# deep-privacy/SA-toolkit

Measured on AMD Instinct MI355X. Metric: anonymized audio seconds per wall-clock second (real-time factor), 5 s @ 16 kHz utterances, higher is better.
Workload: dtype f32 (matrix products as split-f16: hi*hi on the f16 MFMA; cross terms on the block-scaled 8-bit MFMA (weights e4m3, activations e5m2) in the ResBlock convs of stages [1, 2] = 51 % of the generator's FLOP, as two more f16 products elsewhere; f32 accumulate)

## Files before the change

sa-toolkit_amd/csrc/conv1d_mfma.hip:

```cpp
#include "common.h"
#include "conv_common.h"
#include <cstring>

namespace sat {

static int g_k1_gemm = 3;
static int g_lean3 = 1, g_lean7 = 1, g_lean11 = 1;
static int g_trim_halo = 1;
static int g_half_tile7 = 1;
static int g_pair32s = 1;

template <int MT, int NT, int WM, int WN, int KS, bool STRIDE1, int XWI>
__global__ void __launch_bounds__(256, 2) conv1d_mfma_kernel(const ConvArgs p) {
  extern __shared__ __attribute__((aligned(16))) float lds[];
  constexpr int CO_B = 32 * MT * WM;
  constexpr int T_B = 32 * NT * WN;
  static_assert(WM * WN == 4, "4 waves per block");

  const int tid = threadIdx.x;
  const int lane = tid & 63;
  const int wave = tid >> 6;
  const int wm = wave % WM;
  const int wn = wave / WM;
  const int l31 = lane & 31;
// ... 1799 lines not shown
extern "C" int sat_resblock_pair_scaled_f16x3(const sat_conv1d_desc* d, const float* x, const void* w1_packed,
                                              const float* bias1, float w1_descale, const void* w2_packed, float* y, void* stream) {
  SAT_REQUIRE(d && w1_packed && w2_packed && bias1 && d->bias && (x || d->x_split) && (y || (d->no_y && d->y_split)),
              "resblock_pair: null pointer");
  SAT_REQUIRE(d->C_in == d->C_out && d->C_in % 16 == 0 &&
                  (d->C_in <= 32 || (d->C_in == 64 && d->x_split && d->res_split)),
              "resblock_pair: C must be 16 or 32 (64 with 3 taps and split planes end to end)");
  SAT_REQUIRE(d->groups == 1 && d->up == 1 && d->stride == 1 && d->T_q == d->T_in, "resblock_pair: same-length conv pair only");
  SAT_REQUIRE(d->ksize == 3 || d->ksize == 7 || d->ksize == 11, "resblock_pair: kernel size %d not instantiated", d->ksize);
  SAT_REQUIRE(d->in_lrelu, "resblock_pair: both convs take a leaky-relu input");
  SAT_REQUIRE((d->res && d->res == x && !d->res_split) || (!d->res && d->res_split && d->res_split == d->x_split),
              "resblock_pair: the residual is the block input (res == x, or res_split == x_split)");
  ConvArgs a{};
  a.x = x;
  a.w = (const float*)w1_packed;
  a.w2 = w2_packed;
  a.bias1 = bias1;
  a.y = y;
  a.bias = d->bias;
  a.res = d->res;
  a.x_bs = d->x_bstride; a.x_cs = d->x_cstride;
  a.y_bs = d->y_bstride; a.y_cs = d->y_cstride;
  a.r_bs = d->res_bstride; a.r_cs = d->res_cstride;
  a.cin_g = d->C_in; a.cout_g = d->C_out; a.rows_g = d->C_out;
  a.T_in = d->T_in; a.T_q = d->T_q;
  a.ksize = d->ksize; a.dil = d->dilation; a.stride = 1; a.up = 1;
  a.pad_left = (d->ksize * d->dilation - d->dilation) / 2;
  a.cin_pad = round_up(a.cin_g, CI_CHUNK);
  a.co_pad = 64;
  a.w_gs = (long long)(a.cin_pad / CI_CHUNK) * a.ksize * a.co_pad * 64;
  a.in_lrelu = 1; a.in_slope = d->in_slope;
  SAT_REQUIRE(d->in_slope >= 0.f && d->in_slope <= 1.f && (!d->y_split || (d->y_split_slope >= 0.f && d->y_split_slope <= 1.f)) &&
                  (!d->res_split || d->res_split_slope <= 1.f),
              "resblock_pair: leaky-relu slopes must lie in [0, 1] (common.h lrelu_max)");
  a.accum = d->accum; a.accum_div = d->accum_div;
  a.no_store = d->accum_no_store;
  SAT_REQUIRE(!d->accum_no_store || (d->accum && y && d->y_split && !d->no_y), "resblock_pair: accum_no_store goes with accum and y_split");
  a.res_scale = 1.f; a.res_toff = 0; a.res_tstride = 1;
  a.w_descale = d->w_descale != 0.f ? d->w_descale : 1.f;
  a.w_descale1 = w1_descale != 0.f ? w1_descale : 1.f;
  SAT_REQUIRE((long long)a.cin_g * a.x_cs * 4 < (1LL << 31) && (long long)a.rows_g * a.y_cs * 4 < (1LL << 31),
              "resblock_pair: slab too large for 31-bit offsets");
  a.fast_epi = 1;
  a.x16 = d->x_split;
  a.y16 = d->y_split;
  a.y16_slope = d->y_split_slope;
  a.no_y = d->no_y;
  SAT_REQUIRE(!(d->no_y && d->accum), "resblock_pair: no_y with accum");
  if (a.no_y) a.y = (float*)a.y16;
  if (d->res_split) {
    SAT_REQUIRE(d->res_split_slope > 0.f, "resblock_pair: res_split_slope");
    a.res16 = d->res_split;
    a.res16_inv = 1.0f / d->res_split_slope;
  }
  SAT_REQUIRE((long long)a.rows_g * a.T_q * 4 < (1LL << 31), "resblock_pair: slab too large");
  hipStream_t s = (hipStream_t)stream;
  if (a.cin_g == 16 && a.x16 && a.res16) {
    switch (a.ksize) {
      case 3: return launch_pair16<3>(a, d->B, s);
      case 7: return launch_pair16<7>(a, d->B, s);
      default: return launch_pair16<11>(a, d->B, s);
    }
  }
  if (a.cin_g == 64 && g_pair32s && pair32s_supports(a)) return launch_pair32s(a, d->B, s);
  if (a.cin_g == 64) {
    SAT_REQUIRE(pair64_supports(a), "resblock_pair(C = 64): split planes in, residual from planes, (ksize - 1) * dilation <= 64");
    a.xw = g_trim_halo ? 128 + (a.ksize - 1) * a.dil : 192;
    return launch_pair64(a, d->B, s);
  }
  if (a.cin_g == 32 && a.x16 && a.res16) {
    if (g_pair32s && pair32s_supports(a)) return launch_pair32s(a, d->B, s);
    switch (a.ksize) {
      case 3: return launch_pair32<3>(a, d->B, s);
      case 7: return launch_pair32<7>(a, d->B, s);
      default: return launch_pair32<11>(a, d->B, s);
    }
  }
  switch (a.ksize) {
    case 3: return launch_pair<3>(a, d->B, s);
    case 7: return launch_pair<7>(a, d->B, s);
    default: return launch_pair<11>(a, d->B, s);
  }
}

extern "C" int sat_conv1d_f8r_supported(const sat_conv1d_desc* d) {
  if (!d || d->mode != SAT_CONV_F16F8R || !d->x_split || !d->x_split8 || d->groups != 1) return 0;
  ConvArgs a;
  float dummy;
  if (conv1d_prepare(d, nullptr, &dummy, d->no_y ? nullptr : &dummy, a) != SAT_OK) return 0;
  return convring_supports(a, d->B) ? 1 : 0;
}

__global__ void __launch_bounds__(256) planes_f8_sidecar_kernel(const uint4* __restrict__ x, uint4* __restrict__ y, int C, int T) {
  const int t = blockIdx.x * 256 + threadIdx.x;
  const int chunk = blockIdx.y, b = blockIdx.z;
  if (t >= T) return;
  const uint4* xb = x + ((long long)b * (C / 16) + chunk) * 4 * T + t;
  typedef _Float16 h8v __attribute__((ext_vector_type(8)));
  const h8v h0 = __builtin_bit_cast(h8v, xb[0]), h1 = __builtin_bit_cast(h8v, xb[T]);
  const h8v l0 = __builtin_bit_cast(h8v, xb[2LL * T]), l1 = __builtin_bit_cast(h8v, xb[3LL * T]);
  uint4 oh, ol;
  oh.x = pack_e5m2x4((float)h0[0], (float)h0[1], (float)h0[2], (float)h0[3]);
  oh.y = pack_e5m2x4((float)h0[4], (float)h0[5], (float)h0[6], (float)h0[7]);
  oh.z = pack_e5m2x4((float)h1[0], (float)h1[1], (float)h1[2], (float)h1[3]);
  oh.w = pack_e5m2x4((float)h1[4], (float)h1[5], (float)h1[6], (float)h1[7]);
  const float k = F8_XLO_SCALE;
  ol.x = pack_e5m2x4((float)l0[0] * k, (float)l0[1] * k, (float)l0[2] * k, (float)l0[3] * k);
  ol.y = pack_e5m2x4((float)l0[4] * k, (float)l0[5] * k, (float)l0[6] * k, (float)l0[7] * k);
  ol.z = pack_e5m2x4((float)l1[0] * k, (float)l1[1] * k, (float)l1[2] * k, (float)l1[3] * k);
  ol.w = pack_e5m2x4((float)l1[4] * k, (float)l1[5] * k, (float)l1[6] * k, (float)l1[7] * k);
  uint4* yb = y + ((long long)b * (C / 16) + chunk) * 2 * T + t;
  yb[0] = oh;
  yb[T] = ol;
}

extern "C" int sat_planes_f8_sidecar(const void* x_split, void* x_split8, int B, int C, int T, void* stream) {
  SAT_REQUIRE(x_split && x_split8, "planes_f8_sidecar: null pointer");
  SAT_REQUIRE(B > 0 && C > 0 && T > 0 && C % 16 == 0 && B < 65536 && C / 16 < 65536, "planes_f8_sidecar: unsupported shape B=%d C=%d T=%d", B, C, T);
  dim3 grid(ceil_div(T, 256), C / 16, B);
  hipLaunchKernelGGL(planes_f8_sidecar_kernel, grid, dim3(256), 0, (hipStream_t)stream, (const uint4*)x_split, (uint4*)x_split8, C, T);
  SAT_LAUNCH_CHECK("planes_f8_sidecar_kernel");
  return SAT_OK;
}

extern "C" int sat_act_split_f32(const float* x, void* x_split, int B, int C, int T, float slope, int format, void* stream) {
  SAT_REQUIRE(x && x_split, "act_split: null pointer");
  SAT_REQUIRE(format == SAT_SPLIT_F16 || format == SAT_SPLIT_F8, "act_split: unknown format");
  SAT_REQUIRE(B > 0 && C > 0 && T > 0 && C % 16 == 0 && B < 65536, "act_split: unsupported shape B=%d C=%d T=%d", B, C, T);
  SAT_REQUIRE(slope >= 0.f && slope <= 1.f, "act_split: slope must lie in [0, 1]");
  dim3 grid(ceil_div(T, 256), C / 8, B);
  hipLaunchKernelGGL(act_split_kernel, grid, dim3(256), 0, (hipStream_t)stream, x, (uint4*)x_split, C, T, slope, format == SAT_SPLIT_F8);
  SAT_LAUNCH_CHECK("act_split_kernel");
  return SAT_OK;
}

extern "C" int sat_pair32_debug_stamps(int64_t* buf) { return pair32_debug_stamps((long long*)buf); }
extern "C" int sat_convring_debug_stamps(int64_t* buf) { return convring_debug_stamps((long long*)buf); }

extern "C" int sat_conv_set_option(const char* name, int value) {
  SAT_REQUIRE(name, "conv_set_option: null name");
  if (!strcmp(name, "lean3")) { g_lean3 = value != 0; return SAT_OK; }
  if (!strcmp(name, "lean7")) { g_lean7 = value != 0; return SAT_OK; }
  if (!strcmp(name, "lean11")) { g_lean11 = value != 0; return SAT_OK; }
  if (!strcmp(name, "half_tile7")) { g_half_tile7 = value != 0; return SAT_OK; }
  if (!strcmp(name, "pair32s")) { g_pair32s = value != 0; return SAT_OK; }
  if (!strcmp(name, "trim_halo")) { g_trim_halo = value != 0; return SAT_OK; }
  if (!strcmp(name, "pair32w")) { pair32w_set(value); return SAT_OK; }
  if (!strcmp(name, "pair64w")) { pair64w_set(value); return SAT_OK; }
  if (!strcmp(name, "pair64_rpre")) { pair64_rpre_set(value); return SAT_OK; }
  if (!strcmp(name, "convpost_quad")) { convpost_set_quad(value); return SAT_OK; }
  if (!strcmp(name, "convring")) { convring_set(value); return SAT_OK; }
  if (!strcmp(name, "convring_blocks")) { convring_set_blocks(value); return SAT_OK; }
  if (!strcmp(name, "convring_wr")) { convring_set_wr(value); return SAT_OK; }
  if (!strcmp(name, "gemm_walk")) { gemm_walk_set(value); return SAT_OK; }
  if (!strcmp(name, "lean_balance")) { lean_set_balance(value); return SAT_OK; }
  if (!strcmp(name, "pair32s_waves")) { pair32s_set_waves(value); return SAT_OK; }
  if (!strcmp(name, "k1_gemm")) { g_k1_gemm = value < 0 ? 0 : value > 3 ? 3 : value; return SAT_OK; }
  set_error("conv_set_option: unknown option '%s'", name);
  return SAT_ERR_INVALID;
}
```

sa-toolkit_amd/csrc/conv_common.h:

```cpp
#pragma once
#include "common.h"

namespace sat {


typedef float f32x16 __attribute__((ext_vector_type(16)));

typedef int i32x8 __attribute__((ext_vector_type(8)));
typedef _Float16 h8 __attribute__((ext_vector_type(8)));

constexpr float F8_XLO_SCALE = 1024.f;
constexpr int F8_E_XHI = 127, F8_E_XLO = 127 - 10, F8_E_WHI = 127 - 6, F8_E_WLO = 127 - 16;
constexpr int F8R_E_WHI = 127 + 2, F8R_E_WLO = 127 - 9;

__device__ __forceinline__ unsigned pack_e4m3x4(float a, float b, float c, float d) {
  a = __builtin_amdgcn_fmed3f(a, -448.f, 448.f);
  b = __builtin_amdgcn_fmed3f(b, -448.f, 448.f);
  c = __builtin_amdgcn_fmed3f(c, -448.f, 448.f);
  d = __builtin_amdgcn_fmed3f(d, -448.f, 448.f);
  int w = __builtin_amdgcn_cvt_pk_fp8_f32(a, b, 0, false);
  w = __builtin_amdgcn_cvt_pk_fp8_f32(c, d, w, true);
  return (unsigned)w;
}

// ... 441 lines not shown
  const __amdgpu_buffer_rsrc_t scs = __builtin_amdgcn_make_buffer_rsrc((void*)(p.ch_scale ? p.ch_scale : p.y), 0, p.ch_scale ? chn : 0u, 0x00020000);
  const __amdgpu_buffer_rsrc_t shs = __builtin_amdgcn_make_buffer_rsrc((void*)(p.ch_shift ? p.ch_shift : p.y), 0, p.ch_shift ? chn : 0u, 0x00020000);
  const __amdgpu_buffer_rsrc_t y16rs = __builtin_amdgcn_make_buffer_rsrc(
      (void*)(p.y16 ? (char*)p.y16 + (long long)b * p.rows_g * p.T_q * 4 : (char*)p.y), 0,
      p.y16 ? (unsigned)(p.rows_g * p.T_q * 4) : 0u, 0x00020000);
  const int y_rb = (int)p.y_cs * 4;
  const bool has_res = p.res != nullptr || p.res16 != nullptr;
  float bi[MT][4], sc[MT][4], sh[MT][4];
#pragma unroll
  for (int m = 0; m < MT; ++m) {
    const int row0 = co_w + m * 16 + 4 * lg;
#pragma unroll
    for (int r = 0; r < 4; ++r) bi[m][r] = __builtin_bit_cast(float, __builtin_amdgcn_raw_buffer_load_b32(brs, (row0 + r) * 4, 0, 0));
  }
  if (HAS_BN && p.ch_scale) {
#pragma unroll
    for (int m = 0; m < MT; ++m) {
      const int row0 = co_w + m * 16 + 4 * lg;
#pragma unroll
      for (int r = 0; r < 4; ++r) {
        sc[m][r] = __builtin_bit_cast(float, __builtin_amdgcn_raw_buffer_load_b32(scs, (row0 + r) * 4, 0, 0));
        sh[m][r] = __builtin_bit_cast(float, __builtin_amdgcn_raw_buffer_load_b32(shs, (row0 + r) * 4, 0, 0));
      }
    }
  }
  f32x4 yn[NT];
  auto load_accum = [&](int m) __attribute__((always_inline)) {
    const int row0 = co_w + m * 16 + 4 * lg;
#pragma unroll
    for (int n = 0; n < NT; ++n) {
      const int q = q_w + n * 16 + li;
      const unsigned yoff = q < p.T_q ? (unsigned)(row0 * y_rb + q * 4) : OOB;
#pragma unroll
      for (int r = 0; r < 4; ++r) yn[n][r] = __builtin_bit_cast(float, __builtin_amdgcn_raw_buffer_load_b32(yrs, yoff + r * y_rb, 0, 0));
    }
  };
  f32x4 rn[NT];
  if (ROWRES && has_res) epilogue16_load_res_row<NT>(p, rn, b, co_w, q_w, li, lg);
  if (p.accum) load_accum(0);
#pragma unroll
  for (int m = 0; m < MT; ++m) {
    const int row0 = co_w + m * 16 + 4 * lg;
    const bool rows_ok = co_w + m * 16 < p.rows_g;
    f32x4 yv[NT], rr[NT];
    if (ROWRES && has_res) {
#pragma unroll
      for (int n = 0; n < NT; ++n) rr[n] = rn[n];
      if (m + 1 < MT) epilogue16_load_res_row<NT>(p, rn, b, co_w + 16 * (m + 1), q_w, li, lg);
    }
    if (p.accum) {
#pragma unroll
      for (int n = 0; n < NT; ++n) yv[n] = yn[n];
      if (m + 1 < MT) load_accum(m + 1);
    }
#pragma unroll
    for (int n = 0; n < NT; ++n) {
      const int q = q_w + n * 16 + li;
      const bool qok = q < p.T_q;
      const unsigned yoff = qok ? (unsigned)(row0 * y_rb + q * 4) : OOB;
      float rv[4], v[4];
      const f32x4 rw = ROWRES ? rr[n] : rpre[m][n];
      if (p.res16) {
        decode_res16(rw[0], rw[1], rw[2], rw[3], p.res16_inv, rv);
      } else if (p.res) {
#pragma unroll
        for (int r = 0; r < 4; ++r) rv[r] = rw[r];
      }
#pragma unroll
      for (int r = 0; r < 4; ++r) v[r] = __builtin_fmaf(acc[m][n][r], p.w_descale, bi[m][r]);
      if (has_res && !p.res_after) {
#pragma unroll
        for (int r = 0; r < 4; ++r) v[r] += p.res_scale * rv[r];
      }
      if (p.relu && p.relu_first) {
#pragma unroll
        for (int r = 0; r < 4; ++r) v[r] = v[r] > 0.f ? v[r] : 0.f;
      }
      if (HAS_BN && p.ch_scale) {
#pragma unroll
        for (int r = 0; r < 4; ++r) v[r] = v[r] * sc[m][r] + sh[m][r];
      }
      if (p.relu && !p.relu_first) {
#pragma unroll
        for (int r = 0; r < 4; ++r) v[r] = v[r] > 0.f ? v[r] : 0.f;
      }
      if (p.gelu) gelu_fast4(v);
      if (has_res && p.res_after) {
#pragma unroll
        for (int r = 0; r < 4; ++r) v[r] += p.res_scale * rv[r];
      }
      if (p.accum) {
#pragma unroll
        for (int r = 0; r < 4; ++r) v[r] = yv[n][r] + v[r];
      }
      if (p.accum_div != 0.f) {
#pragma unroll
        for (int r = 0; r < 4; ++r) v[r] = v[r] / p.accum_div;
      }
      if (!p.no_y && !p.no_store) {
#pragma unroll
        for (int r = 0; r < 4; ++r)
          __builtin_amdgcn_raw_buffer_store_b32(__builtin_bit_cast(unsigned, v[r]), yrs, yoff + r * y_rb, 0, 0);
      }
      if (p.y16 && rows_ok) {
        const int chunk = (co_w >> 4) + m;
        float u[4];
#pragma unroll
        for (int r = 0; r < 4; ++r) u[r] = lrelu_max(v[r], p.y16_slope);
        const auto h01 = __builtin_amdgcn_cvt_pkrtz(u[0], u[1]);
        const auto h23 = __builtin_amdgcn_cvt_pkrtz(u[2], u[3]);
        const auto l01 = split_lo2(h01, u[0], u[1]);
        const auto l23 = split_lo2(h23, u[2], u[3]);
        const unsigned off = qok ? (unsigned)(((chunk * 4 + (lg >> 1)) * p.T_q + q) * 16 + 8 * (lg & 1)) : OOB;
        typedef unsigned u32x2 __attribute__((ext_vector_type(2)));
        u32x2 hv, lv;
        hv[0] = __builtin_bit_cast(unsigned, h01); hv[1] = __builtin_bit_cast(unsigned, h23);
        lv[0] = __builtin_bit_cast(unsigned, l01); lv[1] = __builtin_bit_cast(unsigned, l23);
        __builtin_amdgcn_raw_buffer_store_b64(hv, y16rs, off, 0, 0);
        __builtin_amdgcn_raw_buffer_store_b64(lv, y16rs, off, 2 * p.T_q * 16, 0);
      }
    }
  }
}

inline bool epilogue16_supports(const ConvArgs& a) {
  return a.fast_epi && !a.y16_f8 && a.up == 1 && !a.poly_planes && a.rows_g % 4 == 0;
}

int launch_f16x3_ring(const ConvArgs& a, int B, hipStream_t s);
int launch_pair64(const ConvArgs& a, int B, hipStream_t s);
bool pair64_supports(const ConvArgs& a);
int launch_pair32s(const ConvArgs& a, int B, hipStream_t s);
bool pair32s_supports(const ConvArgs& a);
void lean_set_balance(int v);
void pair32s_set_waves(int n);
void pair32w_set(int v);
void pair64w_set(int v);
void pair64_rpre_set(int v);
int pair32_debug_stamps(long long* buf);
int launch_f16x3_lean(const ConvArgs& a, int B, hipStream_t s);
bool lean_supports(const ConvArgs& a);
int launch_f16x3_ring16(const ConvArgs& a, int B, hipStream_t s);
int launch_f16x3_convring(const ConvArgs& a, int B, hipStream_t s);
int launch_f16x3_convring_ups(const ConvArgs& a, int B, hipStream_t s);
bool convring_ups_supports(const ConvArgs& a);
int launch_f16x3_convring_multi(const ConvArgs* a, int njobs, int rotate, int B, hipStream_t s);
bool convring_same_shape(const ConvArgs& a, const ConvArgs& b);
bool convring_supports(const ConvArgs& a, int B);
bool convring_wanted(int rows_g, int T_q, int B);
void convring_set(int v);
void convpost_set_quad(int v);
void convring_set_blocks(int v);
void convring_set_wr(int v);
int convring_debug_stamps(long long* buf);
bool ring16_supports(const ConvArgs& a);
int launch_f16x3_gemm_walk(const ConvArgs* a, int njobs, int B, hipStream_t s);
bool gemm_walk_supports(const ConvArgs& a);
bool gemm_walk_same_shape(const ConvArgs& a, const ConvArgs& b);
void gemm_walk_set(int v);
bool gemm_walk_wanted(long long tiles);


}
```

sa-toolkit_amd/csrc/conv_ring16.hip:

```cpp
#include "conv_common.h"

#include <type_traits>

namespace sat {


#define SAT_WAIT_VM(n) asm volatile("s_waitcnt vmcnt(%0)" ::"n"(n) : "memory")
#define SAT_WAIT_VM_LGKM0(n) asm volatile("s_waitcnt vmcnt(%0) lgkmcnt(0)" ::"n"(n) : "memory")

constexpr int CR_STAMPS = 8;
__device__ __forceinline__ long long cr_clock() {
  unsigned long long t;
  asm volatile("s_memtime %0\n\ts_waitcnt lgkmcnt(0)" : "=s"(t)::"memory");
  return (long long)t;
}
__device__ __forceinline__ long long cr_realtime() {
  unsigned long long t;
  asm volatile("s_memrealtime %0\n\ts_waitcnt lgkmcnt(0)" : "=s"(t)::"memory");
  return (long long)t;
}

struct RingJob {
  const void* x16;
  const void* w;
// ... 90 lines not shown
      float v[4];
#pragma unroll
      for (int r = 0; r < 4; ++r) v[r] = __builtin_fmaf(acc[m][n][r], descale, bi[m][r]);
      if (has_res) {
        float rv[4];
        const auto s0 = __builtin_amdgcn_permlane16_swap(rr[n][0], rr[n][2], false, false);
        const auto s1 = __builtin_amdgcn_permlane16_swap(rr[n][1], rr[n][3], false, false);
        rv[0] = mix_add_halves<false>(s0[0], s0[1]);
        rv[1] = mix_add_halves<true>(s0[0], s0[1]);
        rv[2] = mix_add_halves<false>(s1[0], s1[1]);
        rv[3] = mix_add_halves<true>(s1[0], s1[1]);
#pragma unroll
        for (int r = 0; r < 4; ++r) rv[r] = lrelu_undo_min(rv[r], inv);
#pragma unroll
        for (int r = 0; r < 4; ++r) v[r] += rv[r];
      }
      if (accum) {
#pragma unroll
        for (int r = 0; r < 4; ++r) v[r] = yv[n][r] + v[r];
      }
      if (div != 0.f) {
#pragma unroll
        for (int r = 0; r < 4; ++r) v[r] = v[r] / div;
      }
      if (has_y && !no_store) {
        const unsigned yoff = qok ? (unsigned)(row0 * y_rb + q * 4) : OOB;
#pragma unroll
        for (int r = 0; r < 4; ++r) __builtin_amdgcn_raw_buffer_store_b32(__builtin_bit_cast(unsigned, v[r]), yrs, yoff + r * y_rb, 0, 0);
      }
      if (has_y16 && rows_ok) {
        float u[4];
#pragma unroll
        for (int r = 0; r < 4; ++r) u[r] = __builtin_fmaxf(v[r], v[r] * slope);
        const auto h01 = __builtin_amdgcn_cvt_pkrtz(u[0], u[1]);
        const auto h23 = __builtin_amdgcn_cvt_pkrtz(u[2], u[3]);
        const auto l01 = split_lo2(h01, u[0], u[1]);
        const auto l23 = split_lo2(h23, u[2], u[3]);
        const auto s0 = __builtin_amdgcn_permlane16_swap(__builtin_bit_cast(unsigned, h01), __builtin_bit_cast(unsigned, l01), false, false);
        const auto s1 = __builtin_amdgcn_permlane16_swap(__builtin_bit_cast(unsigned, h23), __builtin_bit_cast(unsigned, l23), false, false);
        const u32x4 unit = {s0[0], s1[0], s0[1], s1[1]};
        const unsigned off = (qok && !(hi_only && (lg & 1))) ? (unsigned)(((chunk * 4 + (lg >> 1) + 2 * (lg & 1)) * T_q + q) * 16) : OOB;
        __builtin_amdgcn_raw_buffer_store_b128(unit, y16rs, off, 0, 0);
        if (has_y8) {
          const unsigned x8h = pack_e5m2x4((float)h01[0], (float)h01[1], (float)h23[0], (float)h23[1]);
          const unsigned x8l = pack_e5m2_lo_x4(l01, l23);
          const unsigned off8 = qok ? (unsigned)(((chunk * 2) * T_q + q) * 16 + 4 * lg) : OOB;
          __builtin_amdgcn_raw_buffer_store_b32(x8h, y8rs, off8, 0, 0);
          __builtin_amdgcn_raw_buffer_store_b32(x8l, y8rs, off8, T_q * 16, 0);
        }
      }
    }
  }
}

template <int NT>
__device__ __forceinline__ void ring_epilogue_ups(const RingJob& e, const RingArgs& A, f32x4 (&acc)[4][NT], int b, int co_w, int q_w, int li, int lg) {
  const unsigned OOB = 0x80000000u;
  const int rows_g = A.rows_g, T_q = A.T_q;
  const __amdgpu_buffer_rsrc_t brs = __builtin_amdgcn_make_buffer_rsrc((void*)e.bias, 0, (unsigned)(rows_g), 0x00020000);
  const __amdgpu_buffer_rsrc_t y16rs = __builtin_amdgcn_make_buffer_rsrc((char*)e.y16 + (long long)b * rows_g * T_q * 4, 0, (unsigned)(rows_g * T_q * 4), 0x00020000);
  const __amdgpu_buffer_rsrc_t y8rs = __builtin_amdgcn_make_buffer_rsrc(
      (void*)(e.y8 ? (char*)e.y8 + (long long)b * rows_g * T_q * 2 : (char*)e.bias), 0, e.y8 ? (unsigned)(rows_g * T_q * 2) : 0u, 0x00020000);
  const bool has_y8 = e.y8 != nullptr;
  const float descale = e.w_descale, slope = e.y16_slope;
  typedef unsigned u32x4 __attribute__((ext_vector_type(4)));
  float bi[4];
#pragma unroll
  for (int r = 0; r < 4; ++r) bi[r] = __builtin_bit_cast(float, __builtin_amdgcn_raw_buffer_load_b32(brs, ((co_w >> 2) + 4 * lg + r) * 4, 0, 0));
  if (co_w >= rows_g) return;
  const bool l0 = li & 1, l1 = li & 2;
  const int plane_base = ((co_w >> 6) * 4 + (lg >> 1) + 2 * (lg & 1)) * (4 * T_q);
#pragma unroll
  for (int n = 0; n < NT; ++n) {
    u32x4 un[4];
    unsigned x8[2][4];
#pragma unroll
    for (int m = 0; m < 4; ++m) {
      float u[4];
#pragma unroll
      for (int r = 0; r < 4; ++r) {
        const float v = __builtin_fmaf(acc[m][n][r], descale, bi[r]);
        u[r] = lrelu_max(v, slope);
      }
      const auto h01 = __builtin_amdgcn_cvt_pkrtz(u[0], u[1]);
      const auto h23 = __builtin_amdgcn_cvt_pkrtz(u[2], u[3]);
      const auto l01 = split_lo2(h01, u[0], u[1]);
      const auto l23 = split_lo2(h23, u[2], u[3]);
      const auto s0 = __builtin_amdgcn_permlane16_swap(__builtin_bit_cast(unsigned, h01), __builtin_bit_cast(unsigned, l01), false, false);
      const auto s1 = __builtin_amdgcn_permlane16_swap(__builtin_bit_cast(unsigned, h23), __builtin_bit_cast(unsigned, l23), false, false);
      un[m] = u32x4{s0[0], s1[0], s0[1], s1[1]};
      if (has_y8) {
        x8[0][m] = pack_e5m2x4((float)h01[0], (float)h01[1], (float)h23[0], (float)h23[1]);
        x8[1][m] = pack_e5m2_lo_x4(l01, l23);
      }
    }
    u32x4 p[4], t[4];
#pragma unroll
    for (int w = 0; w < 4; ++w) {
#pragma unroll
      for (int h = 0; h < 2; ++h) {
        const unsigned ev = un[2 * h][w], od = un[2 * h + 1][w];
        const unsigned ev_x = (unsigned)__builtin_amdgcn_mov_dpp((int)ev, 0xB1, 0xF, 0xF, true);
        const unsigned od_x = (unsigned)__builtin_amdgcn_mov_dpp((int)od, 0xB1, 0xF, 0xF, true);
        p[2 * h][w] = l0 ? od_x : ev;
        p[2 * h + 1][w] = l0 ? od : ev_x;
      }
#pragma unroll
      for (int h = 0; h < 2; ++h) {
        const unsigned lo_ = p[h][w], hi_ = p[h + 2][w];
        const unsigned lo_x = (unsigned)__builtin_amdgcn_mov_dpp((int)lo_, 0x4E, 0xF, 0xF, true);
        const unsigned hi_x = (unsigned)__builtin_amdgcn_mov_dpp((int)hi_, 0x4E, 0xF, 0xF, true);
        t[h][w] = l1 ? hi_x : lo_;
        t[h + 2][w] = l1 ? hi_ : lo_x;
      }
    }
#pragma unroll
    for (int j = 0; j < 4; ++j) {
      const int q = q_w + n * 16 + (li & ~3) + j;
      const unsigned off = q < T_q ? (unsigned)((plane_base + 4 * q + (li & 3)) * 16) : OOB;
      __builtin_amdgcn_raw_buffer_store_b128(t[j], y16rs, off, 0, 0);
    }
    if (has_y8) {
#pragma unroll
      for (int term = 0; term < 2; ++term) {
        unsigned p8[4], t8[4];
#pragma unroll
        for (int h = 0; h < 2; ++h) {
          const unsigned ev = x8[term][2 * h], od = x8[term][2 * h + 1];
          const unsigned ev_x = (unsigned)__builtin_amdgcn_mov_dpp((int)ev, 0xB1, 0xF, 0xF, true);
          const unsigned od_x = (unsigned)__builtin_amdgcn_mov_dpp((int)od, 0xB1, 0xF, 0xF, true);
          p8[2 * h] = l0 ? od_x : ev;
          p8[2 * h + 1] = l0 ? od : ev_x;
        }
#pragma unroll
        for (int h = 0; h < 2; ++h) {
          const unsigned lo_ = p8[h], hi_ = p8[h + 2];
          const unsigned lo_x = (unsigned)__builtin_amdgcn_mov_dpp((int)lo_, 0x4E, 0xF, 0xF, true);
          const unsigned hi_x = (unsigned)__builtin_amdgcn_mov_dpp((int)hi_, 0x4E, 0xF, 0xF, true);
          t8[h] = l1 ? hi_x : lo_;
          t8[h + 2] = l1 ? hi_ : lo_x;
        }
        const int base8 = ((co_w >> 6) * 2 + term) * (4 * T_q);
#pragma unroll
        for (int j = 0; j < 4; ++j) {
          const int q = q_w + n * 16 + (li & ~3) + j;
          const unsigned off8 = q < T_q ? (unsigned)((base8 + 4 * q + (li & 3)) * 16 + 4 * lg) : OOB;
          __builtin_amdgcn_raw_buffer_store_b32(t8[j], y8rs, off8, 0, 0);
        }
      }
    }
  }
}

template <int WR, bool STAMP = false, int UMASK = -1, bool F8 = false>
__global__ void __launch_bounds__(512, 2) conv1d_f16x3_ring16_kernel(const RingArgs A, long long* dbg) {
  extern __shared__ __attribute__((aligned(16))) uint4 lds4[];
  static_assert(!(F8 && UMASK >= 0) && !(F8 && WR == 1), "F8: the plain 256 x 160 / 128 x 320 forms only");
  constexpr bool UPS = UMASK >= 0;
  constexpr int WC = 8 / WR, MT = 4, NT = WR == 1 ? 3 : 5, ROWS = 64 * WR, COLS = 16 * NT * WC;
  constexpr int XW = WR == 4 ? 224 : WR == 2 ? 384 : 448;
  constexpr int XP = (XW + 63) / 64;
  constexpr bool XHALF = XW % 64 != 0;
  constexpr int X_UNITS = 8 * XW, W_UNITS = 8 * ROWS, W0 = 2 * X_UNITS;
  constexpr int PW = WR, PX = XP;
  const int tid = threadIdx.x, lane = tid & 63, li = lane & 15, lg = lane >> 4;
  const int wave = __builtin_amdgcn_readfirstlane(tid >> 6);
  const int half = wave >> 2, idx = wave & 3;
  const int wr = WR == 4 ? idx : WR == 2 ? (idx & 1) : 0, wc = WR == 4 ? half : WR == 2 ? ((idx >> 1) + 2 * half) : (idx + 4 * half);
  const int njobs = A.njobs;
  const int nreg = (A.n_vb - (int)blockIdx.x + (int)gridDim.x - 1) / (int)gridDim.x;
  const int ntiles = nreg * njobs;
  long long st_t0 = 0, st_r0 = 0, st_wait = 0, st_pro = 0, st_loop = 0, st_epi = 0;
  if constexpr (STAMP) st_t0 = cr_clock(), st_r0 = cr_realtime();

  struct Tile { int j, b, co_b, q_b; };
  auto locate = [&](int k) __attribute__((always_inline)) {
    Tile t;
    const int i = __builtin_amdgcn_readfirstlane(k / njobs), jj = k - i * njobs;
    const int vb = (int)blockIdx.x + i * (int)gridDim.x;
    const int xcd = vb & 7, rest = vb >> 3;
    const int rt = __builtin_amdgcn_readfirstlane(rest % A.n_rt);
    const int g = __builtin_amdgcn_readfirstlane((rest / A.n_rt) * 8 + xcd);
    t.j = A.rotate ? __builtin_amdgcn_readfirstlane((jj + vb) % njobs) : jj;
    t.b = g < A.total ? __builtin_amdgcn_readfirstlane(g / A.n_ct) : -1;
    t.co_b = rt * ROWS;
    t.q_b = (g - t.b * A.n_ct) * COLS;
    return t;
  };

  i32x4 xrs, wrs;
  int KS = 1, dil = 1, NP = 1, NS = 1, seg_bytes = 0, x_chunk_bytes = 0;
  int ktaps = 1;
  int d_co = 0, d_q0 = 0, d_copad = 0, d_tin = 0;
  const int my_w_unit = half * 4 * ROWS + idx * ROWS, my_x_unit = half * 4 * XW + idx * XW;
  auto setup = [&](const Tile& t) __attribute__((always_inline)) {
    const RingJob p = A.job[t.j];
    KS = p.ksize, dil = p.dil, ktaps = p.ksize;
    NP = A.cin_pad / (2 * CI_CHUNK), NS = F8 ? p.nstep : NP * KS;
    seg_bytes = A.co_pad * 16;
    if (F8 && idx >= 2) {
      x_chunk_bytes = 2 * A.T_in * 16;
      xrs = dma_rsrc((const char*)p.x8 + (long long)t.b * A.cin_g * A.T_in * 2, (unsigned)(A.cin_g * A.T_in * 2));
    } else {
      x_chunk_bytes = 4 * A.T_in * 16;
      xrs = dma_rsrc((const char*)p.x16 + (long long)t.b * A.cin_g * A.T_in * 4, (unsigned)(A.cin_g * A.T_in * 4));
    }
    wrs = dma_rsrc(p.w, p.w_bytes);
    d_co = t.co_b, d_q0 = t.q_b - p.pad_left, d_copad = A.co_pad, d_tin = A.T_in;
  };
  auto voff_w = [&](int j) __attribute__((always_inline)) {
    const int row = d_co + j * 64 + lane;
    return row < d_copad ? (unsigned)(row * 16 + (F8 ? 0 : idx * seg_bytes)) : 0x80000000u;
  };
  auto voff_x = [&](int k) __attribute__((always_inline)) {
    const int xi = d_q0 + k * 64 + lane;
    return (xi >= 0 && xi < d_tin) ? (unsigned)(((F8 ? (idx & 1) : idx) * d_tin + xi) * 16) : 0x80000000u;
  };
  auto issue_w = [&](int pp, int t, int slot) __attribute__((always_inline)) {
    const uint4* dst = lds4 + W0 + slot * W_UNITS + my_w_unit;
    const unsigned soff = F8 ? (unsigned)((t * 8 + wave) * seg_bytes) : (unsigned)((((2 * pp + half) * KS + t) * 4) * seg_bytes);
#pragma unroll
    for (int j = 0; j < PW; ++j) lds_dma16(dst + j * 64, wrs, voff_w(j), soff);
  };
  auto issue_x = [&](int pp) __attribute__((always_inline)) {
    const uint4* dst = lds4 + (pp & 1) * X_UNITS + my_x_unit;
    const unsigned soff = (unsigned)((2 * pp + half) * x_chunk_bytes);
#pragma unroll
    for (int k = 0; k < PX; ++k) {
      if (XHALF && k == PX - 1) lds_dma16_lo32(dst + k * 64, xrs, voff_x(k), soff);
      else lds_dma16(dst + k * 64, xrs, voff_x(k), soff);
    }
  };
  auto issue_prologue = [&]() __attribute__((always_inline)) {
    issue_x(0);
    issue_w(0, 0, 0);
    if (NP > 1) issue_x(1);
    issue_w(0, 1, 1);
    issue_w(0, 2, 2);
  };

  const int a_lane = F8 ? lg * ROWS + wr * 64 + li : (lg >> 1) * 4 * ROWS + (lg & 1) * ROWS + wr * 64 + li;
  const int b_lane = (lg >> 1) * 4 * XW + (lg & 1) * XW + wc * (16 * NT) + li;
  const int b_lane8 = (lg & 1) * 4 * XW + (2 + (lg >> 1)) * XW + wc * (16 * NT) + li;
  const int sc_a = (lg & 1) ? F8R_E_WHI : F8R_E_WLO, sc_b = (lg & 1) ? F8_E_XLO : F8_E_XHI;
  h8 fa[2][MT][2], fb[2][2];
  i32x8 fa8[MT], fb8[2];
  typedef int i32x4v __attribute__((ext_vector_type(4)));
  auto read8 = [&](i32x8& dst, const uint4* p0, const uint4* p1) __attribute__((always_inline)) {
    const i32x4v lo = __builtin_bit_cast(i32x4v, *p0), hi = __builtin_bit_cast(i32x4v, *p1);
    dst = __builtin_shufflevector(lo, hi, 0, 1, 2, 3, 4, 5, 6, 7);
  };
  auto read_a = [&](h8 (&dst)[2], const uint4* wb, int m) __attribute__((always_inline)) {
    dst[0] = __builtin_bit_cast(h8, wb[m * 16]);
    dst[1] = __builtin_bit_cast(h8, wb[m * 16 + (F8 ? 4 : 2) * ROWS]);
  };
  auto read_b = [&](h8 (&dst)[2], const uint4* xb, int n) __attribute__((always_inline)) {
    dst[0] = __builtin_bit_cast(h8, xb[n * 16]);
    dst[1] = __builtin_bit_cast(h8, xb[n * 16 + 2 * XW]);
  };
  f32x4 acc[MT][NT];

  int s = 0, pp = 0, t = 0, ws = 0;
  int p3 = 0, t3 = 0;
  auto body = [&](auto cur, auto late_c, auto more_c, auto tap_c) __attribute__((always_inline)) {
    constexpr int CUR = decltype(cur)::value;
    constexpr int TC = decltype(tap_c)::value;
    constexpr unsigned SK = TC >= 0 ? ((unsigned)UMASK >> (4 * TC)) & 15u : 0u, SK1 = TC >= 0 ? ((unsigned)UMASK >> (4 * ((TC + 1) % 3))) & 15u : 0u;
    constexpr bool LATE = decltype(late_c)::value, MORE = decltype(more_c)::value;
    constexpr int N_HAND = LATE ? NT / 2 : 0;
    constexpr int AR = (MT + NT - 2) / (NT - 1);
    if constexpr (MORE) {
      long long w0 = 0;
      if constexpr (STAMP) w0 = cr_clock();
      if (s + 2 < NS) {
        if (t == 1 && pp >= 1 && pp + 1 < NP) SAT_WAIT_VM_LGKM0(PW + PX);
        else SAT_WAIT_VM_LGKM0(PW);
      } else {
        SAT_WAIT_VM_LGKM0(0);
      }
      asm volatile("s_barrier" ::: "memory");
      if constexpr (STAMP) st_wait += cr_clock() - w0;
    }
    int t1 = t + 1, p1 = pp;
    if (t1 == KS) t1 = 0, p1 = pp + 1;
    const int ws1 = ws == 2 ? 0 : ws + 1;
    const uint4* wnext = lds4 + W0 + ws1 * W_UNITS + a_lane;
    const uint4* xcur = lds4 + (pp & 1) * X_UNITS + b_lane + t * dil;
    const uint4* xnext = lds4 + (p1 & 1) * X_UNITS + b_lane + t1 * dil;
#pragma unroll
    for (int n = 0; n < NT; ++n) {
      __builtin_amdgcn_sched_barrier(0);
      if (n == N_HAND && !(STAMP && (A.diag & 8))) {
        if (t == 0 && pp >= 1 && pp + 1 < NP) issue_x(pp + 1);
        if (s + 3 < NS) issue_w(p3, t3, ws);
      }
      if (!(STAMP && (A.diag & 16))) {
        if (n + 1 < NT) read_b(fb[(n + 1 + CUR) & 1], xcur, n + 1);
        else if constexpr (MORE) read_b(fb[(NT + CUR) & 1], xnext, 0);
        if constexpr (MORE) {
          if (n >= 1) {
#pragma unroll
            for (int m2 = (n - 1) * AR; m2 < n * AR && m2 < MT; ++m2) {
              if ((SK1 >> m2) & 1u) continue;
              read_a(fa[CUR ^ 1][m2], wnext, m2);
            }
          }
        }
      }
      __builtin_amdgcn_sched_barrier(0);
#pragma unroll
      for (int m = 0; m < MT; ++m) {
        if ((SK >> m) & 1u) continue;
        mfma16_acc(acc[m][n], fa[CUR][m][1], fb[(n + CUR) & 1][0]);
        mfma16_acc(acc[m][n], fa[CUR][m][0], fb[(n + CUR) & 1][1]);
        mfma16_acc(acc[m][n], fa[CUR][m][0], fb[(n + CUR) & 1][0]);
      }
    }
    __builtin_amdgcn_sched_barrier(0);
    ++s, pp = p1, t = t1, ws = ws1;
    if (++t3 == KS) t3 = 0, ++p3;
  };
  int e0p = 0, e0t = 0, e1p = 0, e1t = 1;
  int n0p = 0, n0t = 0, n1p = 0, n1t = 0;
  int nxt_x = 2;
  bool xprev = false, fresh = false;
  auto body8 = [&](auto cur, auto late_c, auto more_c) __attribute__((always_inline)) {
    constexpr int CUR = decltype(cur)::value;
    constexpr bool LATE = decltype(late_c)::value, MORE = decltype(more_c)::value;
    constexpr int N_HAND = LATE ? NT / 2 : 0;
    static_assert(MT == NT - 1 || !F8, "one A row of the next step per column 1 .. NT - 1");
    if constexpr (MORE) {
      long long w0 = 0;
      if constexpr (STAMP) w0 = cr_clock();
      if (s + 2 < NS) {
        if (xprev) SAT_WAIT_VM_LGKM0(PW + PX);
        else SAT_WAIT_VM_LGKM0(PW);
      } else {
        SAT_WAIT_VM_LGKM0(0);
      }
      asm volatile("s_barrier" ::: "memory");
      if constexpr (STAMP) st_wait += cr_clock() - w0;
    }
    xprev = false;
    const int ws1 = ws == 2 ? 0 : ws + 1;
    const uint4* wnext = lds4 + W0 + ws1 * W_UNITS + a_lane;
    const int o0 = (e0p & 1) * X_UNITS + e0t * dil, o1 = (e1p & 1) * X_UNITS + e1t * dil;
    const uint4* x16a = lds4 + o0 + b_lane;
    const uint4* x16b = lds4 + o1 + b_lane;
    const uint4* x8a = lds4 + o0 + b_lane8;
    const uint4* x8b = lds4 + o1 + b_lane8;
    const uint4* xn16a = x16a;
    const uint4* xn16b = x16b;
    bool fresh_next = false;
    if constexpr (CUR == 0) {
      if (fresh) {
        fb[0][0] = __builtin_bit_cast(h8, x16a[0]);
        fb[0][1] = __builtin_bit_cast(h8, x16b[0]);
      }
    } else {
      n0p = e1p, n0t = e1t + 1;
      if (n0t == ktaps) n0t = 0, ++n0p;
      n1p = n0p, n1t = n0t + 1;
      if (n1t == ktaps) n1t = 0, ++n1p;
      if (n1p >= NP) n1p = n0p, n1t = n0t;
      if (n0p >= NP) n0p = e1p, n0t = e1t, n1p = e1p, n1t = e1t;
      fresh_next = n1p > e1p;
      xn16a = lds4 + (n0p & 1) * X_UNITS + n0t * dil + b_lane;
      xn16b = lds4 + (n1p & 1) * X_UNITS + n1t * dil + b_lane;
    }
#pragma unroll
    for (int n = 0; n < NT; ++n) {
      __builtin_amdgcn_sched_barrier(0);
      if (n == N_HAND && !(STAMP && (A.diag & 8))) {
        if constexpr (CUR == 0) {
          if (nxt_x < NP && s >= (nxt_x - 1) * ktaps) {
            issue_x(nxt_x);
            ++nxt_x;
            xprev = true;
          }
        }
        if (s + 3 < NS) issue_w(0, s + 3, ws);
      }
      if (!(STAMP && (A.diag & 16))) {
        if constexpr (CUR == 0) {
          if (n + 1 < NT) {
            fb[(n + 1) & 1][0] = __builtin_bit_cast(h8, x16a[(n + 1) * 16]);
            fb[(n + 1) & 1][1] = __builtin_bit_cast(h8, x16b[(n + 1) * 16]);
          } else {
            read8(fb8[0], x8a, x8b);
          }
          if (n >= 1) read8(fa8[n - 1], wnext + (n - 1) * 16, wnext + (n - 1) * 16 + 4 * ROWS);
        } else {
          if (n + 1 < NT) {
            read8(fb8[(n + 1) & 1], x8a + (n + 1) * 16, x8b + (n + 1) * 16);
          } else if constexpr (MORE) {
            if (!fresh_next) {
              fb[0][0] = __builtin_bit_cast(h8, xn16a[0]);
              fb[0][1] = __builtin_bit_cast(h8, xn16b[0]);
            }
          }
          if constexpr (MORE) {
            if (n >= 1) read_a(fa[0][n - 1], wnext, n - 1);
          }
        }
      }
      __builtin_amdgcn_sched_barrier(0);
#pragma unroll
      for (int m = 0; m < MT; ++m) {
        if constexpr (CUR == 0) {
          mfma16_acc(acc[m][n], fa[0][m][0], fb[n & 1][0]);
          mfma16_acc(acc[m][n], fa[0][m][1], fb[n & 1][1]);
        } else {
          mfma8_acc(acc[m][n], fa8[m], fb8[n & 1], sc_a, sc_b);
        }
      }
    }
    __builtin_amdgcn_sched_barrier(0);
    ++s, ws = ws1;
    if constexpr (CUR == 1) e0p = n0p, e0t = n0t, e1p = n1p, e1t = n1t, fresh = fresh_next;
  };
  using I0 = std::integral_constant<int, 0>;
  using I1 = std::integral_constant<int, 1>;
  using I2 = std::integral_constant<int, 2>;
  using NOT = std::integral_constant<int, -1>;
  auto loop = [&](auto late_c) __attribute__((always_inline)) {
    using L = decltype(late_c);
    if constexpr (F8) {
      while (s + 2 < NS) {
        body8(I0{}, L{}, std::true_type{});
        body8(I1{}, L{}, std::true_type{});
      }
      body8(I0{}, L{}, std::true_type{});
      body8(I1{}, L{}, std::false_type{});
    } else if constexpr (UPS) {
      auto six = [&](auto more_last) __attribute__((always_inline)) {
        body(I0{}, L{}, std::true_type{}, I0{});
        body(I1{}, L{}, std::true_type{}, I1{});
        body(I0{}, L{}, std::true_type{}, I2{});
        body(I1{}, L{}, std::true_type{}, I0{});
        body(I0{}, L{}, std::true_type{}, I1{});
        body(I1{}, L{}, more_last, I2{});
      };
      while (s + 6 < NS) six(std::true_type{});
      six(std::false_type{});
    } else {
      while (s + 2 < NS) {
        body(I0{}, L{}, std::true_type{}, NOT{});
        body(I1{}, L{}, std::true_type{}, NOT{});
      }
      body(I0{}, L{}, std::true_type{}, NOT{});
      body(I1{}, L{}, std::false_type{}, NOT{});
    }
  };

  int k = 0;
  Tile cur = locate(0);
  while (k < ntiles && cur.b < 0) cur = locate(++k);
  if (k >= ntiles) return;
  setup(cur);
  issue_prologue();
  while (true) {
    long long e0 = 0;
    if constexpr (STAMP) e0 = cr_clock();
    if (NP > 1) SAT_WAIT_VM(PX + 2 * PW);
    else SAT_WAIT_VM(2 * PW);
    asm volatile("s_barrier" ::: "memory");
#pragma unroll
    for (int m = 0; m < MT; ++m) read_a(fa[0][m], lds4 + W0 + a_lane, m);
    if constexpr (F8) {
      fb[0][0] = __builtin_bit_cast(h8, lds4[b_lane]);
      fb[0][1] = __builtin_bit_cast(h8, lds4[b_lane + (ktaps > 1 ? dil : 0)]);
    } else {
      read_b(fb[0], lds4 + b_lane, 0);
    }
#pragma unroll
    for (int m = 0; m < MT; ++m)
#pragma unroll
      for (int n = 0; n < NT; ++n) acc[m][n] = f32x4{0.f, 0.f, 0.f, 0.f};
    asm volatile("s_nop 3" ::: "memory");
    s = 0, pp = 0, t = 0, ws = 0;
    p3 = KS > 3 ? 0 : 1, t3 = KS > 3 ? 3 : 0;
    e0p = 0, e0t = 0, e1p = 0, e1t = 1, nxt_x = 2, xprev = false, fresh = false;
    if constexpr (STAMP) st_pro += cr_clock() - e0;
    long long l0 = 0;
    if constexpr (STAMP) l0 = cr_clock();
    if (!(A.diag & 2)) {
      if (wave >= 4) loop(std::true_type{});
      else loop(std::false_type{});
    } else {
      asm volatile("s_waitcnt vmcnt(0)" ::: "memory");
    }
    if constexpr (STAMP) st_loop += cr_clock() - l0;
    const Tile done = cur;
    int kn = k + 1;
    Tile nxt = done;
    while (kn < ntiles) {
      nxt = locate(kn);
      if (nxt.b >= 0) break;
      ++kn;
    }
    const bool more = kn < ntiles;
    if (more) {
      asm volatile("s_waitcnt lgkmcnt(0)\n\ts_barrier" ::: "memory");
      setup(nxt);
      issue_prologue();
    }
    long long p0 = 0;
    if constexpr (STAMP) p0 = cr_clock();
    mfma16_drain(acc);
    if (!(A.diag & 4)) {
      const RingJob ej = A.job[done.j];
      if constexpr (UPS) ring_epilogue_ups<NT>(ej, A, acc, done.b, done.co_b + wr * 64, done.q_b + wc * (16 * NT), li, lg);
      else {
        const bool plain = !ej.y && ej.y16 && !ej.accum && ej.accum_div == 0.f && ((ej.y8 != nullptr) == F8);
        const int co_e = done.co_b + wr * 64, q_e = done.q_b + wc * (16 * NT);
        if (plain && !ej.res16 && ((ej.hi_only != 0) == F8)) ring_epilogue<MT, NT, 1, F8>(ej, A, acc, done.b, co_e, q_e, li, lg);
        else if (plain && ej.res16 && !ej.hi_only) ring_epilogue<MT, NT, 2, F8>(ej, A, acc, done.b, co_e, q_e, li, lg);
        else if (ej.y && ej.res16 && !ej.y8) ring_epilogue<MT, NT, 3, F8>(ej, A, acc, done.b, co_e, q_e, li, lg);
        else ring_epilogue<MT, NT>(ej, A, acc, done.b, co_e, q_e, li, lg);
      }
    }
    if constexpr (STAMP) st_epi += cr_clock() - p0;
    if (!more) break;
    k = kn;
    cur = nxt;
  }
  if constexpr (STAMP) {
    if (dbg && (wave & 3) == 0 && lane == 0) {
      long long* d = dbg + ((long long)blockIdx.x * 2 + half) * CR_STAMPS;
      const long long t_end = cr_clock(), r_end = cr_realtime();
      d[0] = st_pro;
      d[1] = st_loop;
      d[2] = st_wait;
      d[3] = st_epi;
      d[4] = t_end - st_t0;
      d[5] = r_end - st_r0;
      d[6] = st_r0;
      d[7] = ntiles;
    }
  }
}

static int g_convring = 1;
void convring_set(int v) { g_convring = v; }
static int g_convring_blocks = 0;
void convring_set_blocks(int v) { g_convring_blocks = v < 0 ? 0 : v / 8 * 8; }
static long long* g_convring_dbg = nullptr;
int convring_debug_stamps(long long* buf) {
  g_convring_dbg = buf;
  return CR_STAMPS;
}

static int cu_count() {
  static std::atomic<int> n{0};
  int v = n.load(std::memory_order_relaxed);
  if (!v) {
    int dev = 0;
    hipDeviceProp_t pr;
    if (hipGetDevice(&dev) == hipSuccess && hipGetDeviceProperties(&pr, dev) == hipSuccess) v = pr.multiProcessorCount;
    if (v <= 0) v = 256;
    n.store(v, std::memory_order_relaxed);
  }
  return v;
}

bool convring_supports(const ConvArgs& a, int B) {
  if (!(g_convring & 1) && !a.f8r) return false;
  if (!(a.x16 && !a.f8 && !a.y16_f8 && !a.poly_planes && !a.k1_wrap && a.fast_epi && a.up == 1 && a.stride == 1)) return false;
  if (a.f8r && !a.x8) return false;
  if (a.y8 && !a.y16) return false;
  if (a.y16 && !(a.y16_slope > 0.f && a.y16_slope <= 1.f)) return false;
  if (a.res16 && !(a.res16_inv >= 1.f)) return false;
  if (!epilogue16_supports(a) || a.ksize < 3 || a.cin_g % 32 != 0 || a.rows_g <= 64) return false;
  if (a.ch_scale || a.relu || a.gelu || a.res || a.res_after || !a.bias || (a.res16 && a.res_scale != 1.f) || (a.accum && a.no_y)) return false;
  const int halo = (a.ksize - 1) * a.dil;
  if (halo > 64) return false;
  if (!a.f8r && ((a.cin_pad / (2 * CI_CHUNK)) * a.ksize) % 2 != 0) return false;
  const long long tiles = a.rows_g > 128 ? (long long)ceil_div(a.rows_g, 256) * ceil_div(a.T_q, 160) * B
                          : a.rows_g > 64 ? (long long)ceil_div(a.T_q, 320) * B : (long long)ceil_div(a.T_q, 384) * B;
  return a.f8r || (g_convring & 32) || tiles * 4 >= (long long)cu_count() * 3;
}

bool convring_wanted(int rows_g, int T_q, int B) {
  if (!(g_convring & 1) || rows_g <= 64) return false;
  const long long tiles = rows_g > 128 ? (long long)ceil_div(rows_g, 256) * ceil_div(T_q, 160) * B : (long long)ceil_div(T_q, 320) * B;
  return (g_convring & 32) || tiles * 4 >= (long long)cu_count() * 3;
}

bool convring_same_shape(const ConvArgs& a, const ConvArgs& b) {
  return a.cin_g == b.cin_g && a.cin_pad == b.cin_pad && a.rows_g == b.rows_g && a.co_pad == b.co_pad && a.T_in == b.T_in && a.T_q == b.T_q &&
         a.f8r == b.f8r;
}

bool convring_ups_supports(const ConvArgs& a) {
  if (!(a.x16 && a.y16 && a.no_y && !a.f8 && !a.f8r && !a.y16_f8 && !a.k1_wrap && a.up == 4 && a.stride == 1)) return false;
  if (a.ksize != 3 || a.cin_g % 64 != 0 || a.cin_pad != a.cin_g || a.rows_g <= 128 || a.rows_g % 64 != 0 || !a.bias) return false;
  if (a.ch_scale || a.relu || a.gelu || a.res || a.res16 || a.res_after || a.accum) return false;
  return (a.ksize - 1) * a.dil <= 64;
}

template <int WR, int UMASK = -1, bool F8 = false>
static int launch_convring(const ConvArgs* a, int njobs, int rotate, int B, hipStream_t s) {
  constexpr int WC = 8 / WR, NT = WR == 1 ? 3 : 5, ROWS = 64 * WR, COLS = 16 * NT * WC, XW = WR == 4 ? 224 : WR == 2 ? 384 : 448;
  RingArgs A{};
  for (int j = 0; j < njobs; ++j) {
    RingJob& r = A.job[j];
    r.x16 = a[j].x16, r.w = a[j].w, r.bias = a[j].bias;
    r.y = a[j].no_y ? nullptr : a[j].y;
    r.y16 = a[j].y16, r.res16 = a[j].res16;
    r.w_descale = a[j].w_descale, r.y16_slope = a[j].y16_slope, r.res16_inv = a[j].res16_inv, r.accum_div = a[j].accum_div;
    r.ksize = a[j].ksize, r.dil = a[j].dil, r.pad_left = a[j].pad_left, r.accum = a[j].accum;
    r.w_bytes = (unsigned)a[j].w_gs;
    r.y_bs = a[j].y_bs, r.y_cs = a[j].y_cs;
    r.x8 = a[j].x8, r.y8 = a[j].y8, r.hi_only = a[j].y16_hi_only && a[j].y8;
    r.no_store = a[j].no_store;
    r.nstep = F8 ? 2 * (((a[j].cin_pad / (2 * CI_CHUNK)) * a[j].ksize + 1) / 2) : a[j].ksize;
  }
  A.cin_g = a[0].cin_g, A.cin_pad = a[0].cin_pad, A.rows_g = a[0].rows_g, A.co_pad = a[0].co_pad, A.T_in = a[0].T_in, A.T_q = a[0].T_q;
  A.njobs = njobs;
  A.rotate = rotate && njobs > 1;
  A.diag = g_convring & 30;
  A.n_rt = ceil_div(a[0].rows_g, ROWS);
  A.n_ct = ceil_div(a[0].T_q, COLS);
  A.total = A.n_ct * B;
  A.n_vb = 8 * A.n_rt * ceil_div(A.total, 8);
  const size_t lds_bytes = ((size_t)2 * 8 * XW + (size_t)3 * 8 * ROWS) * 16;
  const int grid = std::min(A.n_vb, std::max(8, (g_convring_blocks ? std::min(g_convring_blocks, cu_count()) : cu_count()) / 8 * 8));
  auto kern = conv1d_f16x3_ring16_kernel<WR, false, UMASK, F8>;
  auto kern_st = conv1d_f16x3_ring16_kernel<WR, UMASK < 0, UMASK, F8>;
  static std::atomic<uint64_t> attr_done{0};
  int dev;
  if (attr_needed_on_current_device(attr_done, &dev)) {
    SAT_HIP(hipFuncSetAttribute((const void*)kern, hipFuncAttributeMaxDynamicSharedMemorySize, (int)lds_bytes));
    SAT_HIP(hipFuncSetAttribute((const void*)kern_st, hipFuncAttributeMaxDynamicSharedMemorySize, (int)lds_bytes));
    attr_done_on_device(attr_done, dev);
  }
  if (g_convring_dbg) hipLaunchKernelGGL(kern_st, dim3(grid), dim3(512), lds_bytes, s, A, g_convring_dbg);
  else hipLaunchKernelGGL(kern, dim3(grid), dim3(512), lds_bytes, s, A, (long long*)nullptr);
  SAT_LAUNCH_CHECK(F8 ? "conv1d_f16x3_ring16_kernel (F8: 8-bit cross terms)" : "conv1d_f16x3_ring16_kernel");
  return SAT_OK;
}

static int g_convring_wr = 0;
void convring_set_wr(int v) { g_convring_wr = v; }
int launch_f16x3_convring_multi(const ConvArgs* a, int njobs, int rotate, int B, hipStream_t s) {
  if (a[0].f8r) return a[0].rows_g > 128 && !(g_convring_wr & 2) ? launch_convring<4, -1, true>(a, njobs, rotate, B, s) : launch_convring<2, -1, true>(a, njobs, rotate, B, s);
  return a[0].rows_g > 128 && !(g_convring_wr & 1) ? launch_convring<4>(a, njobs, rotate, B, s) : launch_convring<2>(a, njobs, rotate, B, s);
}

int launch_f16x3_convring(const ConvArgs& a, int B, hipStream_t s) { return launch_f16x3_convring_multi(&a, 1, 0, B, s); }

constexpr unsigned UPS_MASK_K8 = 0x30cu;
int launch_f16x3_convring_ups(const ConvArgs& a, int B, hipStream_t s) {
  return a.up_zero_taps == UPS_MASK_K8 ? launch_convring<4, (int)UPS_MASK_K8>(&a, 1, 0, B, s) : launch_convring<4, 0>(&a, 1, 0, B, s);
}

}
```

Baseline: 15590.

## Add four-slot weight ring for F8 convring with one barrier per tap pair

Adds a TP variant of the ring16 conv kernel for the F8 cross-term path. It uses four LDS weight slots instead of three, prefetches two weight steps at once, and barriers only on every other step, so block-wide synchronisation happens once per tap pair. The variant becomes the default for f8r convs and always uses the 128x320 tile form, dropping the 256-row tile choice. In exchange it takes more LDS (160 KiB), which may limit occupancy, and it waits for all outstanding loads (vmcnt 0) at each barrier.

Measured after the change: 15660 (median of 4 runs). Within noise of the previous version (+0.4%).

```diff
diff --git a/sa-toolkit_amd/csrc/conv1d_mfma.hip b/sa-toolkit_amd/csrc/conv1d_mfma.hip
--- a/sa-toolkit_amd/csrc/conv1d_mfma.hip
+++ b/sa-toolkit_amd/csrc/conv1d_mfma.hip
@@ -1975,6 +1975,7 @@
   if (!strcmp(name, "convring")) { convring_set(value); return SAT_OK; }
   if (!strcmp(name, "convring_blocks")) { convring_set_blocks(value); return SAT_OK; }
   if (!strcmp(name, "convring_wr")) { convring_set_wr(value); return SAT_OK; }
+  if (!strcmp(name, "convring_f8_ring3")) { convring_set_f8_ring3(value); return SAT_OK; }
   if (!strcmp(name, "gemm_walk")) { gemm_walk_set(value); return SAT_OK; }
   if (!strcmp(name, "lean_balance")) { lean_set_balance(value); return SAT_OK; }
   if (!strcmp(name, "pair32s_waves")) { pair32s_set_waves(value); return SAT_OK; }
diff --git a/sa-toolkit_amd/csrc/conv_common.h b/sa-toolkit_amd/csrc/conv_common.h
--- a/sa-toolkit_amd/csrc/conv_common.h
+++ b/sa-toolkit_amd/csrc/conv_common.h
@@ -617,6 +617,7 @@
 void convpost_set_quad(int v);
 void convring_set_blocks(int v);
 void convring_set_wr(int v);
+void convring_set_f8_ring3(int v);
 int convring_debug_stamps(long long* buf);
 bool ring16_supports(const ConvArgs& a);
 int launch_f16x3_gemm_walk(const ConvArgs* a, int njobs, int B, hipStream_t s);
diff --git a/sa-toolkit_amd/csrc/conv_ring16.hip b/sa-toolkit_amd/csrc/conv_ring16.hip
--- a/sa-toolkit_amd/csrc/conv_ring16.hip
+++ b/sa-toolkit_amd/csrc/conv_ring16.hip
@@ -266,10 +266,11 @@
   }
 }
 
-template <int WR, bool STAMP = false, int UMASK = -1, bool F8 = false>
-__global__ void __launch_bounds__(512, 2) conv1d_f16x3_ring16_kernel(const RingArgs A, long long* dbg) {
+template <int WR, bool STAMP, int UMASK, bool F8, bool TP>
+__device__ __forceinline__ void ring16_walk(const RingArgs& A, long long* dbg) {
   extern __shared__ __attribute__((aligned(16))) uint4 lds4[];
   static_assert(!(F8 && UMASK >= 0) && !(F8 && WR == 1), "F8: the plain 256 x 160 / 128 x 320 forms only");
+  static_assert(!TP || (F8 && WR == 2), "TP: the F8 form on 128 x 320 tiles (four W slots: 160 KiB of LDS)");
   constexpr bool UPS = UMASK >= 0;
   constexpr int WC = 8 / WR, MT = 4, NT = WR == 1 ? 3 : 5, ROWS = 64 * WR, COLS = 16 * NT * WC;
   constexpr int XW = WR == 4 ? 224 : WR == 2 ? 384 : 448;
@@ -443,20 +444,24 @@
     constexpr bool LATE = decltype(late_c)::value, MORE = decltype(more_c)::value;
     constexpr int N_HAND = LATE ? NT / 2 : 0;
     static_assert(MT == NT - 1 || !F8, "one A row of the next step per column 1 .. NT - 1");
-    if constexpr (MORE) {
+    if constexpr (MORE && !(TP && CUR == 1)) {
       long long w0 = 0;
       if constexpr (STAMP) w0 = cr_clock();
-      if (s + 2 < NS) {
-        if (xprev) SAT_WAIT_VM_LGKM0(PW + PX);
-        else SAT_WAIT_VM_LGKM0(PW);
+      if constexpr (TP) {
+        SAT_WAIT_VM_LGKM0(0);
       } else {
-        SAT_WAIT_VM_LGKM0(0);
+        if (s + 2 < NS) {
+          if (xprev) SAT_WAIT_VM_LGKM0(PW + PX);
+          else SAT_WAIT_VM_LGKM0(PW);
+        } else {
+          SAT_WAIT_VM_LGKM0(0);
+        }
       }
       asm volatile("s_barrier" ::: "memory");
       if constexpr (STAMP) st_wait += cr_clock() - w0;
     }
     xprev = false;
-    const int ws1 = ws == 2 ? 0 : ws + 1;
+    const int ws1 = TP ? (ws + 1) & 3 : ws == 2 ? 0 : ws + 1;
     const uint4* wnext = lds4 + W0 + ws1 * W_UNITS + a_lane;
     const int o0 = (e0p & 1) * X_UNITS + e0t * dil, o1 = (e1p & 1) * X_UNITS + e1t * dil;
     const uint4* x16a = lds4 + o0 + b_lane;
@@ -485,7 +490,19 @@
 #pragma unroll
     for (int n = 0; n < NT; ++n) {
       __builtin_amdgcn_sched_barrier(0);
-      if (n == N_HAND && !(STAMP && (A.diag & 8))) {
+      if constexpr (TP) {
+        if (!(STAMP && (A.diag & 8))) {
+          if constexpr (CUR == 0) {
+            if (n == N_HAND && nxt_x < NP && s >= (nxt_x - 1) * ktaps) {
+              issue_x(nxt_x);
+              ++nxt_x;
+            }
+          } else {
+            if (n == N_HAND && s + 2 < NS) issue_w(0, s + 2, (s + 2) & 3);
+            if (n == N_HAND + 1 && s + 3 < NS) issue_w(0, s + 3, (s + 3) & 3);
+          }
+        }
+      } else if (!TP && n == N_HAND && !(STAMP && (A.diag & 8))) {
         if constexpr (CUR == 0) {
           if (nxt_x < NP && s >= (nxt_x - 1) * ktaps) {
             issue_x(nxt_x);
@@ -655,6 +672,15 @@
   }
 }
 
+template <int WR, bool STAMP = false, int UMASK = -1, bool F8 = false>
+__global__ void __launch_bounds__(512, 2) conv1d_f16x3_ring16_kernel(const RingArgs A, long long* dbg) {
+  ring16_walk<WR, STAMP, UMASK, F8, false>(A, dbg);
+}
+template <bool STAMP = false>
+__global__ void __launch_bounds__(512, 2) conv1d_f16x3_ring16_kernel_tp(const RingArgs A, long long* dbg) {
+  ring16_walk<2, STAMP, -1, true, true>(A, dbg);
+}
+
 static int g_convring = 1;
 void convring_set(int v) { g_convring = v; }
 static int g_convring_blocks = 0;
@@ -713,7 +739,7 @@
   return (a.ksize - 1) * a.dil <= 64;
 }
 
-template <int WR, int UMASK = -1, bool F8 = false>
+template <int WR, int UMASK = -1, bool F8 = false, bool TP = false>
 static int launch_convring(const ConvArgs* a, int njobs, int rotate, int B, hipStream_t s) {
   constexpr int WC = 8 / WR, NT = WR == 1 ? 3 : 5, ROWS = 64 * WR, COLS = 16 * NT * WC, XW = WR == 4 ? 224 : WR == 2 ? 384 : 448;
   RingArgs A{};
@@ -738,10 +764,10 @@
   A.n_ct = ceil_div(a[0].T_q, COLS);
   A.total = A.n_ct * B;
   A.n_vb = 8 * A.n_rt * ceil_div(A.total, 8);
-  const size_t lds_bytes = ((size_t)2 * 8 * XW + (size_t)3 * 8 * ROWS) * 16;
+  const size_t lds_bytes = ((size_t)2 * 8 * XW + (size_t)(TP ? 4 : 3) * 8 * ROWS) * 16;
   const int grid = std::min(A.n_vb, std::max(8, (g_convring_blocks ? std::min(g_convring_blocks, cu_count()) : cu_count()) / 8 * 8));
-  auto kern = conv1d_f16x3_ring16_kernel<WR, false, UMASK, F8>;
-  auto kern_st = conv1d_f16x3_ring16_kernel<WR, UMASK < 0, UMASK, F8>;
+  auto kern = TP ? conv1d_f16x3_ring16_kernel_tp<false> : conv1d_f16x3_ring16_kernel<WR, false, UMASK, F8>;
+  auto kern_st = TP ? conv1d_f16x3_ring16_kernel_tp<true> : conv1d_f16x3_ring16_kernel<WR, UMASK < 0, UMASK, F8>;
   static std::atomic<uint64_t> attr_done{0};
   int dev;
   if (attr_needed_on_current_device(attr_done, &dev)) {
@@ -751,14 +777,21 @@
   }
   if (g_convring_dbg) hipLaunchKernelGGL(kern_st, dim3(grid), dim3(512), lds_bytes, s, A, g_convring_dbg);
   else hipLaunchKernelGGL(kern, dim3(grid), dim3(512), lds_bytes, s, A, (long long*)nullptr);
-  SAT_LAUNCH_CHECK(F8 ? "conv1d_f16x3_ring16_kernel (F8: 8-bit cross terms)" : "conv1d_f16x3_ring16_kernel");
+  SAT_LAUNCH_CHECK(TP   ? "conv1d_f16x3_ring16_kernel_tp (F8: 8-bit cross terms, one barrier per tap pair)"
+                   : F8 ? "conv1d_f16x3_ring16_kernel (F8: 8-bit cross terms)"
+                        : "conv1d_f16x3_ring16_kernel");
   return SAT_OK;
 }
 
 static int g_convring_wr = 0;
 void convring_set_wr(int v) { g_convring_wr = v; }
+static int g_convring_f8_ring3 = 0;
+void convring_set_f8_ring3(int v) { g_convring_f8_ring3 = v != 0; }
 int launch_f16x3_convring_multi(const ConvArgs* a, int njobs, int rotate, int B, hipStream_t s) {
-  if (a[0].f8r) return a[0].rows_g > 128 && !(g_convring_wr & 2) ? launch_convring<4, -1, true>(a, njobs, rotate, B, s) : launch_convring<2, -1, true>(a, njobs, rotate, B, s);
+  if (a[0].f8r) {
+    if (!g_convring_f8_ring3) return launch_convring<2, -1, true, true>(a, njobs, rotate, B, s);
+    return a[0].rows_g > 128 && !(g_convring_wr & 2) ? launch_convring<4, -1, true>(a, njobs, rotate, B, s) : launch_convring<2, -1, true>(a, njobs, rotate, B, s);
+  }
   return a[0].rows_g > 128 && !(g_convring_wr & 1) ? launch_convring<4>(a, njobs, rotate, B, s) : launch_convring<2>(a, njobs, rotate, B, s);
 }
 
```
